# theovincent/iS-DQN

Hardware: AMD Instinct MI355X
Metric: gradient-steps/sec (batch=256, K=9, 84x84x4) (higher is better)
Workload: dtype bf16x3 (split-bf16 MFMA operands hi+lo, fp32 accumulate)

## Files before the change

### is-dqn_amd/csrc/conv_img.h

```cpp
#pragma once
#include "net_problems.h"

namespace isdqn {

__device__ __forceinline__ int column_slot(int c16) { return c16 < 4 ? 8 + c16 : (c16 < 12 ? c16 - 4 : c16); }
struct PixelOrder {
    int strips;
    int n_full;
    int full_w;
    FastDiv d_h8, d_rem, d_w;
    PixelOrder() : strips(0), n_full(0), full_w(0) {}
    PixelOrder(int H, int W, bool use_strips) : strips(use_strips ? 1 : 0), n_full(H * 8 * (W / 8)), full_w(8 * (W / 8)) {
        d_h8 = FastDiv((uint32_t)(H * 8));
        d_rem = FastDiv((uint32_t)(W % 8 ? W % 8 : 1));
        d_w = FastDiv((uint32_t)W);
    }
    __device__ __forceinline__ void map(int n, int& y, int& x) const {
        uint32_t a, b;
        if (!strips) {
            d_w.divmod((uint32_t)n, a, b);
            y = (int)a; x = (int)b;
        } else if (n < n_full) {
            d_h8.divmod((uint32_t)n, a, b);
            y = (int)(b >> 3); x = (int)(a * 8 + (b & 7));
// ... 553 lines not shown
#undef ISDQN_STAMP
#undef ISDQN_ABLATED
}

template <int MT, int PASSES, bool U8, int KG = 1>
static int launch_conv_fwd_img(const ConvImgParams& p, hipStream_t st) {
    using T = ConvImgTraits<MT, PASSES, U8>;
    const int lds = (KG * 2 * T::A_STAGE + T::B_PLANES * p.plane_elems) * 2;
    static LdsConfigured configured;
    if (int rc = ensure_dynamic_lds(&conv_fwd_img_kernel<MT, PASSES, U8, KG>, lds, configured)) return rc;
    ISDQN_REPORT_OCCUPANCY((&conv_fwd_img_kernel<MT, PASSES, U8, KG>), GEMM_THREADS * KG, lds, p.n_img * p.tiles_per_img);
    hipLaunchKernelGGL((conv_fwd_img_kernel<MT, PASSES, U8, KG>), dim3(p.n_img * p.tiles_per_img), dim3(GEMM_THREADS * KG), lds,
                       st, p);
    ISDQN_HIP_CHECK(hipGetLastError());
    return ISDQN_OK;
}

static inline int conv_img_geometry(const ConvGeom& g, bool u8, int stack, int b_planes, int mt, int a_planes, int& R,
                                    int& Wp, int& plane_elems, int pixel_pitch = 0) {
    int rows_per_tile = g.npix <= 128 ? g.hout : ((128 + g.wout - 2) / g.wout + 1);
    if (rows_per_tile > g.hout) rows_per_tile = g.hout;
    R = g.stride * (rows_per_tile - 1) + g.ksz;
    if (u8) {
        Wp = ((g.wout - 1) * g.stride + g.ksz + 7) / 8 * 8;
        plane_elems = stack * R * Wp;
    } else {
        Wp = (g.wout - 1) * g.stride + g.ksz;
        plane_elems = R * Wp * (pixel_pitch ? pixel_pitch : g.cin_p);
    }
    const int a_stage = a_planes * (mt * 16) * 48;
    return (2 * a_stage + b_planes * plane_elems) * 2;
}


struct ConvWgradImgParams {
    ConvGeom g;
    const float* dz;
    const float* in;
    FrameSrc fs;
    float* slabs;
    float scale;
    int n_img, G;
    int n_col_groups, NC;
    int R, Wp;
    int PPin;
    int in_plane;
    int PA, npix_pad;
    int dz_plane;
    FastDiv d_ncg;
    FastDiv d_chunk, d_Wp, d_R, d_dzchunk, d_npixpad;
    int prefetch;
    long long* stamps;
};
template <int WV> struct WgradPrefetch { static constexpr int DZ = 1024 / (64 * WV), IN = WV == 4 ? 6 : 5, DZ_U8 = 1792 / (64 * WV); };

template <bool U8, int PASSES, int NTHR = GEMM_THREADS>
__device__ __forceinline__ void fill_input_image(__bf16* img, int plane_elems, const ConvGeom& g, const FrameSrc& fs,
                                                 const float* in, int j, int row_base, int R, int Wp, int PP, int tid,
                                                 const FastDiv& d_chunk, const FastDiv& d_Wp, const FastDiv& d_R) {
    constexpr int FILL_BATCH = 8;
    if constexpr (U8) {
        fill_frames_u8<NTHR>(img, fs, j, row_base, -g.pad, R, Wp, tid, d_chunk);
    } else {
        fill_image_s8<NTHR, (PASSES >= 3 ? 2 : 1), FILL_BATCH>(img, plane_elems, in + (int64_t)j * g.hin * g.win * g.cin_p, g.hin, g.win, g.cin_p,
                                                               row_base, -g.pad, R, Wp, PP, tid, d_chunk, d_Wp);
    }
}

__device__ __forceinline__ bf16x8 tr_frag(const __bf16* a0, const __bf16* a1) {
    s16x4 lo = __builtin_amdgcn_ds_read_tr16_b64_v4i16((LDS_AS s16x4*)a0);
    s16x4 hi = __builtin_amdgcn_ds_read_tr16_b64_v4i16((LDS_AS s16x4*)a1);
    s16x8 r = __builtin_shufflevector(lo, hi, 0, 1, 2, 3, 4, 5, 6, 7);
    return __builtin_bit_cast(bf16x8, r);
}

template <int MT, int NTW, int PASSES, bool U8, int WV = 4>
__global__ __launch_bounds__(64 * WV) void conv_wgrad_img_kernel(const ConvWgradImgParams p) {
    ISDQN_EMPTY_KERNEL_RETURN
    constexpr int NTHR = 64 * WV;
    constexpr int A_PLANES = PASSES >= 2 ? 2 : 1;
    constexpr int B_PLANES = (PASSES >= 3) ? 2 : 1;
    extern __shared__ __attribute__((aligned(16))) char smem_raw[];
    __bf16* dzi = reinterpret_cast<__bf16*>(smem_raw);
    __bf16* img = dzi + A_PLANES * p.dz_plane;
    const ConvGeom& g = p.g;
    const int tid = threadIdx.x, lane = tid & 63, wave = tid >> 6;
#if defined(ISDQN_DEV)
#define WG_STAMP(i)                                                                                   \
    if (p.stamps != nullptr && threadIdx.x == 0) {                                                   \
        p.stamps[(int64_t)blockIdx.x * 8 + (i)] = (long long)__builtin_amdgcn_s_memtime();            \
        if ((i) == 0) p.stamps[(int64_t)blockIdx.x * 8 + 7] = (long long)__builtin_amdgcn_s_memrealtime(); \
    }
#else
#define WG_STAMP(i)
#endif
    WG_STAMP(0);
    uint32_t ig_u, cg_u;
    p.d_ncg.divmod(blockIdx.x, ig_u, cg_u);
    const int cg = (int)cg_u, ig = (int)ig_u;
    const int j0 = ig * p.G, j1 = min(p.n_img, j0 + p.G);
    const int grp = lane >> 4, li = lane & 15, q = li >> 2, pq = li & 3;

    int col_off[NTW];
#pragma unroll
    for (int t = 0; t < NTW; ++t) {
        const int c0 = cg * p.NC + (wave + WV * t) * 16;
        if constexpr (U8) {
            const int c = c0 >> 6, ky0 = (c0 >> 3) & 7;
            col_off[t] = (c * p.R + ky0 + (pq >> 1)) * p.Wp + 4 * (pq & 1);
        } else {
            uint32_t tap, ci, ky, kx;
            g.d_cinp.divmod((uint32_t)(c0 < g.K ? c0 : 0), tap, ci);
            g.d_ksz.divmod(tap, ky, kx);
            col_off[t] = ((int)ky * p.Wp + (int)kx) * p.PPin + (int)ci + 4 * pq;
        }
    }

    f32x4 acc[MT][NTW];
#pragma unroll
    for (int mt = 0; mt < MT; ++mt)
#pragma unroll
        for (int t = 0; t < NTW; ++t) mfma_init(acc[mt][t]);

    const int nsteps = p.npix_pad / GEMM_BK;
    auto k_steps = [&]() {
        for (int ks = 0; ks < nsteps; ++ks) {
            int pixoff[2], arow[2];
#pragma unroll
            for (int h = 0; h < 2; ++h) {
                int kp = ks * GEMM_BK + tr_row(8 * grp + 4 * h + q);
                arow[h] = kp * p.PA + 4 * pq;
                kp = kp < g.npix ? kp : g.npix - 1;
                uint32_t oy, ox;
                g.d_wout.divmod((uint32_t)kp, oy, ox);
                pixoff[h] = U8 ? ((int)oy * g.stride * p.Wp + (int)ox * g.stride)
                               : ((int)oy * g.stride * p.Wp + (int)ox * g.stride) * p.PPin;
            }
            bf16x8 fa_hi[MT], fa_lo[MT];
#pragma unroll
            for (int mt = 0; mt < MT; ++mt) {
                fa_hi[mt] = tr_frag(dzi + arow[0] + mt * 16, dzi + arow[1] + mt * 16);
                if constexpr (PASSES >= 2)
                    fa_lo[mt] = tr_frag(dzi + p.dz_plane + arow[0] + mt * 16, dzi + p.dz_plane + arow[1] + mt * 16);
            }
#pragma unroll
            for (int t = 0; t < NTW; ++t) {
                const __bf16* b0 = img + pixoff[0] + col_off[t];
                const __bf16* b1 = img + pixoff[1] + col_off[t];
                bf16x8 fb_hi = tr_frag(b0, b1), fb_lo;
                if constexpr (PASSES >= 3) fb_lo = tr_frag(b0 + p.in_plane, b1 + p.in_plane);
#pragma unroll
// ... 31 lines not shown
                if (j == j0) { WG_STAMP(2); } else if (j == j0 + 1) { WG_STAMP(4); }
            }
        }
    }
    if (!staged)
    for (int j = j0; j < j1; ++j) {
        __syncthreads();
        bool dz_done = false;
        if constexpr (U8) {
            if (p.prefetch) {
                ImagePrefetch<WgradPrefetch<WV>::DZ_U8> ra;
                request_image_s8<NTHR>(ra, p.dz + (int64_t)j * g.npix * g.cout_p, 1, g.npix, g.cout_p, 0, 0, 1, p.npix_pad, p.PA, tid,
                                       p.d_dzchunk, p.d_npixpad);
                fill_input_image<U8, PASSES, NTHR>(img, p.in_plane, g, p.fs, p.in, j, -g.pad, p.R, p.Wp, p.PPin, tid, p.d_chunk, p.d_Wp, p.d_R);
                commit_image_s8<A_PLANES>(dzi, p.dz_plane, ra);
                dz_done = true;
            }
        }
        if (!dz_done) {
            fill_image_s8<NTHR, A_PLANES, 8>(dzi, p.dz_plane, p.dz + (int64_t)j * g.npix * g.cout_p, 1, g.npix, g.cout_p, 0, 0, 1, p.npix_pad,
                                             p.PA, tid, p.d_dzchunk, p.d_npixpad);
            fill_input_image<U8, PASSES, NTHR>(img, p.in_plane, g, p.fs, p.in, j, -g.pad, p.R, p.Wp, p.PPin, tid, p.d_chunk, p.d_Wp, p.d_R);
        }
        __syncthreads();
        if (j == j0) { WG_STAMP(1); } else if (j == j0 + 1) { WG_STAMP(3); }
        k_steps();
        if (j == j0) { WG_STAMP(2); } else if (j == j0 + 1) { WG_STAMP(4); }
    }

    float* slab = p.slabs + (int64_t)ig * g.cout_p * g.K;
#pragma unroll
    for (int mt = 0; mt < MT; ++mt)
#pragma unroll
        for (int t = 0; t < NTW; ++t) {
            const int col = cg * p.NC + (wave + WV * t) * 16 + li;
#pragma unroll
            for (int r = 0; r < 4; ++r) {
                const int row = mt * 16 + grp * 4 + r;
#if !defined(ISDQN_NO_STREAMING)
                if (row < g.cout_p && col < g.K) __builtin_nontemporal_store(acc[mt][t][r] * p.scale, (ISDQN_GLOBAL float*)(slab + (int64_t)row * g.K + col));
#else
                if (row < g.cout_p && col < g.K) slab[(int64_t)row * g.K + col] = acc[mt][t][r] * p.scale;
#endif
            }
        }
#if defined(ISDQN_DEV)
    if (p.stamps != nullptr) {
        __builtin_amdgcn_s_waitcnt(0);
        WG_STAMP(5);
    }
#endif
#undef WG_STAMP
}

template <int MT, int NTW, int PASSES, bool U8, int WV = 4>
static int launch_conv_wgrad_img(const ConvWgradImgParams& p, int n_img_groups, hipStream_t st) {
    constexpr int A_PLANES = PASSES >= 2 ? 2 : 1;
    constexpr int B_PLANES = (PASSES >= 3) ? 2 : 1;
    const int lds = (A_PLANES * p.dz_plane + B_PLANES * p.in_plane) * 2;
    static LdsConfigured configured;
    if (int rc = ensure_dynamic_lds(&conv_wgrad_img_kernel<MT, NTW, PASSES, U8, WV>, lds, configured)) return rc;
    ISDQN_REPORT_OCCUPANCY((&conv_wgrad_img_kernel<MT, NTW, PASSES, U8, WV>), 64 * WV, lds, n_img_groups * p.n_col_groups);
    ConvWgradImgParams q = p;
    q.prefetch = 0;
#if !defined(ISDQN_WGRAD_NO_PREFETCH)
    if (!U8 && p.G >= 2 && p.npix_pad * (p.g.cout_p / 8) <= WgradPrefetch<WV>::DZ * 64 * WV &&
        p.R * p.Wp * (p.g.cin_p / 8) <= WgradPrefetch<WV>::IN * 64 * WV)
        q.prefetch = 1;
#if !defined(ISDQN_WGRAD_NO_U8_DZ)
    if (U8 && p.npix_pad * (p.g.cout_p / 8) <= WgradPrefetch<WV>::DZ_U8 * 64 * WV) q.prefetch = 1;
#endif
#endif
    hipLaunchKernelGGL((conv_wgrad_img_kernel<MT, NTW, PASSES, U8, WV>), dim3(n_img_groups * p.n_col_groups),
                       dim3(64 * WV), lds, st, q);
    ISDQN_HIP_CHECK(hipGetLastError());
    return ISDQN_OK;
}


struct ConvDgradImgParams {
    ConvGeom g;
    const float* W;
    const float* dz;
    const float* z_in;
    const float *gamma, *beta;
    int c_in;
    float* dz_in;
    float* part;
    int n_img, T, Kc;
    int Hd, Wd, PPd, bt;
    FastDiv d_chunk, d_Wd, d_T;
    long long* stamps;
    int dz_plane;
    int tiles_per_img;
    int cls_tile_start[5];
    PixelOrder cls_order[4];
    int n_classes;
};

template <int MT, int PASSES, int NT = 2>
__global__ __launch_bounds__(GEMM_THREADS, 2) void conv_dgrad_img_kernel(const ConvDgradImgParams p) {
    ISDQN_EMPTY_KERNEL_RETURN
    constexpr int BM = MT * 16;
    constexpr int A_PLANES = PASSES >= 2 ? 2 : 1;
    constexpr int B_PLANES = PASSES >= 3 ? 2 : 1;
    using GA = TileGeom<BM, true>;
    constexpr int A_STAGE = A_PLANES * GA::ELEMS;
    extern __shared__ __attribute__((aligned(16))) char smem_raw[];
    __bf16* a_stage = reinterpret_cast<__bf16*>(smem_raw);
    __bf16* img = a_stage + 2 * A_STAGE;
    __shared__ float s_part[4][3][64];
    const ConvGeom& g = p.g;
    const int tid = threadIdx.x, lane = tid & 63, wave = tid >> 6, grp = lane >> 4;
#if defined(ISDQN_DEV)
#define ISDQN_STAMP(i)                                                                               \
    if (p.stamps != nullptr && threadIdx.x == 0) {                                                  \
        p.stamps[(int64_t)blockIdx.x * 8 + (i)] = (long long)__builtin_amdgcn_s_memtime();           \
        if ((i) == 0) p.stamps[(int64_t)blockIdx.x * 8 + 7] = (long long)__builtin_amdgcn_s_memrealtime(); \
    }
#define ISDQN_ABLATED(bit) ((p.ablate & (bit)) != 0)
#else
#define ISDQN_STAMP(i)
#define ISDQN_ABLATED(bit) (false)
#endif
    ISDQN_STAMP(0);

    int j, tl;
// ... 298 lines not shown
                    out[mt][r] = ok ? rstd * (gg[mt][r] - m1 - xh[mt][r] * m2) : 0.f;
                    dbias[mt][r] += out[mt][r];
                }
        } else {
#pragma unroll
            for (int mt = 0; mt < MT; ++mt)
#pragma unroll
                for (int r = 0; r < 4; ++r) {
                    const bool ok = pix_ok[nt] && (mt * 16 + grp * 4 + r) < p.c_in;
                    out[mt][r] = (ok && zv[mt][r] > 0.f) ? acc[mt][nt][r] : 0.f;
                    dbias[mt][r] += out[mt][r];
                }
        }
        if (pix_ok[nt]) {
#pragma unroll
            for (int mt = 0; mt < MT; ++mt) {
                const int ch0 = mt * 16 + grp * 4;
                if (ch0 < g.cin_p)
                    s8_store_quad_paired(p.dz_in + pixel * g.cin_p, ch0, out[mt][0], out[mt][1], out[mt][2], out[mt][3]);
            }
        }
    }
#pragma unroll
    for (int mt = 0; mt < MT; ++mt)
#pragma unroll
        for (int r = 0; r < 4; ++r) {
            dg[mt][r] = row16_sum(dg[mt][r]);
            db[mt][r] = row16_sum(db[mt][r]);
            dbias[mt][r] = row16_sum(dbias[mt][r]);
            if ((lane & 15) == 0) {
                const int ch = mt * 16 + grp * 4 + r;
                s_part[wave][0][ch] = dg[mt][r];
                s_part[wave][1][ch] = db[mt][r];
                s_part[wave][2][ch] = dbias[mt][r];
            }
        }
    __syncthreads();
    for (int i = tid; i < 3 * g.cin_p; i += GEMM_THREADS) {
        const int which = (i >= g.cin_p) + (i >= 2 * g.cin_p), c = i - which * g.cin_p;
        p.part[((int64_t)blockIdx.x * 3 + which) * g.cin_p + c] =
            s_part[0][which][c] + s_part[1][which][c] + s_part[2][which][c] + s_part[3][which][c];
    }
    ISDQN_STAMP(4);
#if defined(ISDQN_DEV)
    if (p.stamps != nullptr) {
        __builtin_amdgcn_s_waitcnt(0);
        ISDQN_STAMP(5);
    }
#endif
#undef ISDQN_STAMP
#undef ISDQN_ABLATED
}

constexpr int REDUCE_MAX_JOBS = 4;
struct ReduceJobs {
    const float* part[REDUCE_MAX_JOBS];
    float* out[REDUCE_MAX_JOBS];
    int n_rows[REDUCE_MAX_JOBS], width[REDUCE_MAX_JOBS];
    int block_start[REDUCE_MAX_JOBS + 1];
    int n;
};
__global__ __launch_bounds__(256) void reduce_rows_kernel(const ReduceJobs jobs) {
    ISDQN_EMPTY_KERNEL_RETURN
    __shared__ float s_red[32][8];
    int job = 0;
#pragma unroll
    for (int i = 1; i < REDUCE_MAX_JOBS; ++i)
        if (i < jobs.n && (int)blockIdx.x >= jobs.block_start[i]) job = i;
    const float* __restrict__ part = jobs.part[job];
    float* __restrict__ out = jobs.out[job];
    const int n_rows = jobs.n_rows[job], width = jobs.width[job];
    const int col = ((int)blockIdx.x - jobs.block_start[job]) * 8 + (threadIdx.x & 7), rl = threadIdx.x >> 3;
    float s = 0.f;
    if (col < width) {
        int r = rl;
        for (; r + 7 * 32 < n_rows; r += 8 * 32) {
            float v[8];
#pragma unroll
            for (int u = 0; u < 8; ++u) v[u] = part[(int64_t)(r + u * 32) * width + col];
#pragma unroll
            for (int u = 0; u < 8; ++u) s += v[u];
        }
        for (; r < n_rows; r += 32) s += part[(int64_t)r * width + col];
    }
    s_red[rl][threadIdx.x & 7] = s;
    __syncthreads();
    if (rl == 0 && col < width) {
        float t = 0.f;
#pragma unroll
        for (int k = 0; k < 32; ++k) t += s_red[k][threadIdx.x & 7];
        out[col] = t;
    }
}

template <int MT, int PASSES, int NT = 2>
static int launch_conv_dgrad_img(const ConvDgradImgParams& p, hipStream_t st) {
    constexpr int A_PLANES = PASSES >= 2 ? 2 : 1;
    constexpr int B_PLANES = PASSES >= 3 ? 2 : 1;
    using GA = TileGeom<MT * 16, true>;
    const int lds = (2 * A_PLANES * GA::ELEMS + B_PLANES * p.dz_plane) * 2;
    static LdsConfigured configured;
    if (int rc = ensure_dynamic_lds(&conv_dgrad_img_kernel<MT, PASSES, NT>, lds, configured)) return rc;
    ISDQN_REPORT_OCCUPANCY((&conv_dgrad_img_kernel<MT, PASSES, NT>), GEMM_THREADS, lds, p.n_img * p.tiles_per_img);
    hipLaunchKernelGGL((conv_dgrad_img_kernel<MT, PASSES, NT>), dim3(p.n_img * p.tiles_per_img), dim3(GEMM_THREADS), lds, st, p);
    ISDQN_HIP_CHECK(hipGetLastError());
    return ISDQN_OK;
}

}
```

### is-dqn_amd/csrc/net_kernels.hip

```cpp
#include <stdarg.h>
#include <stdlib.h>

#include <algorithm>
#include <type_traits>
#include <vector>
#include <atomic>

#include "conv_img.h"
#include "conv_u8_pair.h"
#include "conv_s8_pair.h"
#include "munchausen.h"
#include "hl_gauss.h"
#include "quantile.h"
#include "net_plan.h"
#include "net_problems.h"

namespace isdqn {

__device__ inline double pow_int(double b, int t) {
    double r = 1.0, x = b;
    for (unsigned u = (unsigned)t; u != 0; u >>= 1) {
        if (u & 1u) r *= x;
        x *= x;
    }
// ... 1344 lines not shown
    else if (Cp <= 128) LAUNCH_SMALL(32);
    else if (Cp <= 256) LAUNCH_SMALL(64);
    else {
        ISDQN_REQUIRE(Cp <= 256 * LN_WIDE_MAX_COLS, ISDQN_ERR_UNSUPPORTED, "hidden dense width above 4096");
        nb = rows < LN_MAX_BLOCKS ? rows : LN_MAX_BLOCKS;
        hipLaunchKernelGGL(ln_bwd_wide_kernel, dim3(nb), dim3(256), 0, st, da, z, gamma, beta, rows, C, Cp, dz, part);
    }
#undef LAUNCH_SMALL
    ISDQN_HIP_CHECK(hipGetLastError());
    *n_blocks_out = nb;
    return ISDQN_OK;
}

template <int BM, int PASSES>
static int launch_conv_dgrad(const Layer& l, const float* wmir, const float* dz, float* da, int n_img,
                             hipStream_t st) {
    ConvDgrad<BM, PASSES> p;
    p.g = conv_geom(l);
    p.W = wmir + l.w_off;
    p.dz = dz; p.da = da; p.n_img = n_img;
    p.T = l.ksz / l.stride;
    p.Kc = p.T * p.T * l.cout_p;
    p.n_classes = l.stride * l.stride;
    int acc = 0;
    for (int c = 0; c < p.n_classes; ++c) {
        int cy = c / l.stride, cx = c % l.stride;
        int Ha = (l.hin - cy + l.stride - 1) / l.stride, Wb = (l.win - cx + l.stride - 1) / l.stride;
        p.tile_start[c] = acc;
        p.cls_d_hw[c] = FastDiv((uint32_t)(Ha * Wb));
        p.cls_d_w[c] = FastDiv((uint32_t)Wb);
        acc += ceil_div(n_img * Ha * Wb, 128);
    }
    p.tile_start[p.n_classes] = acc;
    return launch_gemm(p, acc, st);
}

template <int PASSES, bool U8>
static int launch_conv_wgrad(const Layer& l, const NetInput& in, const float* act_in, const float* dz, float* slabs,
                             int n_img, hipStream_t st) {
    ConvWgrad<PASSES, U8> p;
    p.g = conv_geom(l);
    p.n_pix = n_img * l.npix;
    p.DZ = MatSrc{dz, l.cout_p, p.n_pix, l.cout_p, 1};
    p.in = act_in;
    p.fs = FrameSrc{in.frames, in.frame_stride, in.frame_ids, l.cin, in.paired_B, l.hin, l.win, in.id_pitch, in.id_off};
    p.slabs = slabs;
    p.scale = U8 ? (1.0f / 255.0f) : 1.0f;
    p.tiles_n = ceil_div(l.K, 64);
    int ksteps = ceil_div(p.n_pix, GEMM_BK);
    p.steps_per_split = ceil_div(ksteps, l.gw_slabs);
    p.splits = ceil_div(ksteps, p.steps_per_split);
    return launch_gemm(p, p.tiles_n * p.splits, st);
}
static int conv_wgrad_img(const Layer& l, bool x3, const NetInput& in, const float* act_in, const float* dz, float* slabs,
                          int n_img, hipStream_t st, int* slabs_out) {
    *slabs_out = 0;
    if (!l.wgi_ntw || n_img != 0 && ceil_div(n_img, l.wgi_G) > l.gw_slabs) return ISDQN_OK;
    ConvWgradImgParams wp;
    wp.g = conv_geom(l);
    const int passes = x3 ? (l.is_u8 ? 2 : 3) : 1;
    const int mt = l.cout_p <= 32 ? 2 : 4;
    int lds_unused_R, Wp, plane;
    conv_img_geometry(wp.g, l.is_u8, l.cin, 1, mt, 1, lds_unused_R, Wp, plane);
    wp.R = l.stride * (l.hout - 1) + l.ksz;
    wp.Wp = Wp;
    wp.PPin = l.cin_p;
    for (int pad = 0; pad <= 24; pad += 8)
        if ((l.stride * (l.cin_p + pad)) % 32 == 16) { wp.PPin = l.cin_p + pad; break; }
    wp.in_plane = l.is_u8 ? l.cin * wp.R * Wp : wp.R * Wp * wp.PPin;
    wp.PA = l.cout_p + (l.cout_p % 32 == 0 ? 16 : 8);
    wp.npix_pad = round_up(l.npix, 32);
    wp.dz_plane = wp.npix_pad * wp.PA;
    const int lds = ((passes >= 2 ? 2 : 1) * wp.dz_plane + (passes >= 3 ? 2 : 1) * wp.in_plane) * 2;
    if (lds > 150 * 1024 || (l.is_u8 && (l.win < 8 || l.cin > 4))) return ISDQN_OK;
    wp.d_chunk = FastDiv((uint32_t)(l.is_u8 ? Wp / 8 : l.cin_p / 8));
    wp.d_Wp = FastDiv((uint32_t)Wp);
    wp.d_R = FastDiv((uint32_t)wp.R);
    wp.d_dzchunk = FastDiv((uint32_t)(l.cout_p / 8));
    wp.d_npixpad = FastDiv((uint32_t)wp.npix_pad);
    wp.dz = dz; wp.in = act_in;
    wp.fs = FrameSrc{in.frames, in.frame_stride, in.frame_ids, l.cin, in.paired_B, l.hin, l.win, in.id_pitch, in.id_off};
    wp.slabs = slabs;
    wp.scale = l.is_u8 ? (1.0f / 255.0f) : 1.0f;
    wp.n_img = n_img; wp.G = l.wgi_G;
    wp.NC = 64 * l.wgi_ntw;
    wp.n_col_groups = l.K / wp.NC;
    wp.d_ncg = FastDiv((uint32_t)wp.n_col_groups);
    {
        char tag[32];
        snprintf(tag, sizeof(tag), "wgrad:%s", l.name);
        wp.stamps = stamps_for(tag);
    }
    const int groups = ceil_div(n_img, l.wgi_G);
    *slabs_out = groups;
#define WGI(MT_, NTW_, P_, U_) return launch_conv_wgrad_img<MT_, NTW_, P_, U_>(wp, groups, st)
#define WGI8(MT_, NTW_, P_, U_) return launch_conv_wgrad_img<MT_, NTW_, P_, U_, 8>(wp, groups, st)
    if (l.is_u8) {
        if (mt == 2) { if (l.wgi_ntw == 4) { if (passes == 2) WGI(2, 4, 2, true); else WGI(2, 4, 1, true); }
                       if (l.wgi_ntw == 2) { if (passes == 2) WGI(2, 2, 2, true); else WGI(2, 2, 1, true); } }
        else         { if (l.wgi_ntw == 4) { if (passes == 2) WGI(4, 4, 2, true); else WGI(4, 4, 1, true); }
                       if (l.wgi_ntw == 2) { if (passes == 2) WGI(4, 2, 2, true); else WGI(4, 2, 1, true); } }
    } else {
        if (mt == 2) { if (l.wgi_ntw == 4) { if (passes == 3) WGI(2, 4, 3, false); else WGI(2, 4, 1, false); }
                       if (l.wgi_ntw == 3) { if (passes == 3) WGI(2, 3, 3, false); else WGI(2, 3, 1, false); }
                       if (l.wgi_ntw == 2) { if (passes == 3) WGI(2, 2, 3, false); else WGI(2, 2, 1, false); } }
        else         {
                       static const bool w4 = ISDQN_DEV_ENV("ISDQN_WGRAD_4WAVES");
                       if (l.wgi_ntw == 8 && !w4) { if (passes == 3) WGI8(4, 4, 3, false); else WGI8(4, 4, 1, false); }
                       if (l.wgi_ntw == 9) { if (passes == 3) WGI(4, 9, 3, false); else WGI(4, 9, 1, false); }
                       if (l.wgi_ntw == 8) { if (passes == 3) WGI(4, 8, 3, false); else WGI(4, 8, 1, false); }
                       if (l.wgi_ntw == 4) { if (passes == 3) WGI(4, 4, 3, false); else WGI(4, 4, 1, false); }
                       if (l.wgi_ntw == 3) { if (passes == 3) WGI(4, 3, 3, false); else WGI(4, 3, 1, false); }
                       if (l.wgi_ntw == 2) { if (passes == 3) WGI(4, 2, 3, false); else WGI(4, 2, 1, false); } }
    }
#undef WGI
#undef WGI8
    *slabs_out = 0;
    return ISDQN_OK;
}

static void add_reduce_job(ReduceJobs& jobs, const float* part, int n_rows, int width, float* out) {
    const int i = jobs.n++;
    jobs.part[i] = part; jobs.out[i] = out; jobs.n_rows[i] = n_rows; jobs.width[i] = width;
    jobs.block_start[i + 1] = jobs.block_start[i] + ceil_div(width, 8);
}

static int conv_dgrad_img(const Layer& l, const Layer& below, bool x3, const float* params, const float* wmir, const float* dz, float* ws,
                          int n_img, hipStream_t st, bool* done, ReduceJobs* jobs) {
    *done = false;
    if (!l.dgi_tiles || below.part_rows < n_img * l.dgi_tiles) return ISDQN_OK;
    ConvDgradImgParams dp;
    dp.g = conv_geom(l);
    dp.W = wmir + l.w_off;
    dp.dz = dz;
    dp.z_in = ws + below.z_off;
    dp.gamma = below.has_ln ? params + below.g_off : nullptr;
    dp.beta = below.has_ln ? params + below.be_off : nullptr;
    dp.c_in = below.out_f;
    dp.dz_in = ws + below.dz_off;
    dp.part = ws + below.part_off;
    dp.n_img = n_img;
    dp.T = l.ksz / l.stride;
    dp.Kc = dp.T * dp.T * l.cout_p;
#if defined(ISDQN_DGRAD_WIDE_BORDER)
    dp.bt = dp.T - 1;
#else
    dp.bt = dp.T - 1 - l.pad / l.stride > 0 ? dp.T - 1 - l.pad / l.stride : 0;
#endif
    const int need_h = (l.hin - 1 + l.pad) / l.stride + 1, need_w = (l.win - 1 + l.pad) / l.stride + 1;
    dp.Hd = dp.bt + (l.hout > need_h ? l.hout : need_h);
    dp.Wd = dp.bt + (l.wout > need_w ? l.wout : need_w);
    dp.PPd = l.cout_p + ((16 - l.cout_p % 32) + 32) % 32;
    dp.dz_plane = dp.Hd * dp.Wd * dp.PPd;
    dp.d_chunk = FastDiv((uint32_t)(l.cout_p / 8));
    dp.d_Wd = FastDiv((uint32_t)dp.Wd);
    dp.d_T = FastDiv((uint32_t)dp.T);
    {
        char tag[32];
        snprintf(tag, sizeof(tag), "dgrad:%s", l.name);
        dp.stamps = stamps_for(tag);
    }
    dp.n_classes = l.stride * l.stride;
    int acc = 0;
    for (int c = 0; c < dp.n_classes; ++c) {
        int cy = c / l.stride, cx = c % l.stride;
        int Ha = (l.hin - cy + l.stride - 1) / l.stride, Wb = (l.win - cx + l.stride - 1) / l.stride;
        dp.cls_tile_start[c] = acc;
        dp.cls_order[c] = PixelOrder(Ha, Wb, Ha * Wb <= 128);
        acc += ceil_div(Ha * Wb, l.dgi_tile_pix);
    }
    dp.cls_tile_start[dp.n_classes] = acc;
// ... 527 lines not shown

struct WgradJob {
    int layer = -1;
    hipStream_t stream = nullptr;
    hipEvent_t wait = nullptr;
    const float* dz = nullptr;
    int dz_ld = 0;
};

static int dense_wgrad_fused_adam(const LearnCtx& c, const Layer& l, const float* act_in, const WgradJob& j) {
    const MatSrc A{j.dz, j.dz_ld, c.B, l.out_p, 1};
    const MatSrc Bm{act_in, l.in_p, c.B, l.in_p, 1};
    AdamFuse af{c.params + l.w_off, c.adam_m + l.w_off, c.adam_v + l.w_off, c.ws + c.P.adam_tab_off,
                c.cfg->learning_rate, c.cfg->adam_b1, c.cfg->adam_b2, c.cfg->adam_eps,
                c.grad_out ? c.grad_out + l.w_off : nullptr, c.ws + c.P.wsplit_off + l.w_off, c.update ? 1 : 0};
    if (l.is_head)
        return c.x3 ? launch_plain<64, 64, 2, 2, true, true, 3, true, false, true, 2>(A, nullptr, 0, Bm, nullptr, l.in_p, l.out_p, l.in_p, c.B, 1, 0,
                                                                                      j.stream, &af)
                    : launch_plain<64, 64, 2, 2, true, true, 1, true, false, true, 2>(A, nullptr, 0, Bm, nullptr, l.in_p, l.out_p, l.in_p, c.B, 1, 0,
                                                                                      j.stream, &af);
    return c.x3 ? launch_plain<64, 64, 2, 2, true, true, 3, true, false, true, DZ_S8 | 2>(A, nullptr, 0, Bm, nullptr, l.in_p, l.out_p, l.in_p, c.B, 1,
                                                                                          0, j.stream, &af)
                : launch_plain<64, 64, 2, 2, true, true, 1, true, false, true, DZ_S8 | 2>(A, nullptr, 0, Bm, nullptr, l.in_p, l.out_p, l.in_p, c.B, 1,
                                                                                          0, j.stream, &af);
}

static int weight_gradient(const LearnCtx& c, const WgradJob& j, AdamList* adam) {
    const Layer& l = c.P.L[j.layer];
    float* ws = c.ws;
    const float* act_in = j.layer > 0 ? ws + c.P.L[j.layer - 1].act_off : nullptr;
    int w_slabs, rc;
    if (l.is_head && c.hc_S && c.ss) {
        w_slabs = effective_splits(c.B, l.gw_slabs);
    } else if (l.kind == 0) {
        rc = conv_wgrad(l, c.x3, c.in, act_in, j.dz, ws + l.gw_off, c.B, j.stream, &w_slabs);
        if (rc) return rc;
    } else {
        w_slabs = effective_splits(c.B, l.gw_slabs);
        if (w_slabs == 1 && !l.in_unpadded_ld) return dense_wgrad_fused_adam(c, l, act_in, j);
        rc = dense_wgrad(l, c.x3, c.in, act_in, j.dz, j.dz_ld, ws + l.gw_off, c.B, j.stream);
        if (rc) return rc;
    }
    adam[c.ss && j.stream == c.wst ? 1 : 0].add(l.w_off, l.w_size, ws + l.gw_off, w_slabs, l.w_size);
    return ISDQN_OK;
}

#if !defined(ISDQN_FORK_LATE_MAX_B)
#define ISDQN_FORK_LATE_MAX_B 768
#endif
struct BackwardSchedule {
    const LearnCtx& c;
    AdamList* const adam;
    const bool tail_swap, fork_late;
    bool prio_pending, head_pending;
    hipEvent_t head_event = nullptr;
    bool forked = false, layer0_chained = false;
    WgradJob deferred;

    BackwardSchedule(const LearnCtx& ctx, AdamList* lists)
        : c(ctx), adam(lists), tail_swap(ctx.ss && ctx.P.n_layers >= 3 && !ctx.P.L[1].is_head),
          fork_late(ctx.ss != nullptr && ctx.P.L[0].kind != 2 && ctx.B <= ISDQN_FORK_LATE_MAX_B),
          prio_pending(ctx.batch->priorities_ready != nullptr), head_pending(ctx.hc_S && ctx.ss) {}

    bool wgrad_on_side(int i) const { return c.ss && !c.P.L[i].is_head && (tail_swap ? i != 1 : i > 0); }
    hipStream_t wgrad_stream(int i) const { return wgrad_on_side(i) || (c.P.L[i].is_head && c.hc_S) ? c.wst : c.st; }
    bool forks_after_dgrad(int i) const { return wgrad_on_side(i) && c.P.L[i].kind == 1 && i > 0; }
    bool forks_before_dgrad(int i) const { return wgrad_on_side(i) && !forks_after_dgrad(i) && !(i == 0 && layer0_chained); }
    bool adam_on_side() const { return c.ss && forked && tail_swap; }

    int signal_priorities() {
        if (prio_pending) {
            prio_pending = false;
            ISDQN_HIP_CHECK(hipEventRecord((hipEvent_t)c.batch->priorities_ready, c.st));
        }
        return ISDQN_OK;
    }
    int run_head_tail(hipStream_t s) {
        if (!head_pending) return ISDQN_OK;
        head_pending = false;
        return head_chain_tail(c, s);
    }
    int begin() {
        if (!c.ss)
            if (int rc = signal_priorities()) return rc;
        if (fork_late && head_pending) {
            head_event = next_event(c.ss);
            ISDQN_HIP_CHECK(hipEventRecord(head_event, c.st));
        }
        return ISDQN_OK;
    }
    int fork(hipStream_t side) {
        if (int rc = chain(c.ss, c.st, side)) return rc;
        if (int rc = signal_priorities()) return rc;
        forked = true;
        return deferred.layer < 0 ? run_head_tail(side) : ISDQN_OK;
    }
    int fork_after_dgrad(WgradJob& job, bool* defer) {
        if (!fork_late) {
            if (int rc = chain(c.ss, c.st, job.stream)) return rc;
            if (int rc = signal_priorities()) return rc;
            forked = true;
            return run_head_tail(job.stream);
        }
        if (head_event != nullptr && head_pending) {
            ISDQN_HIP_CHECK(hipStreamWaitEvent(job.stream, head_event, 0));
            if (int rc = run_head_tail(job.stream)) return rc;
        }
        job.wait = next_event(c.ss);
        ISDQN_HIP_CHECK(hipEventRecord(job.wait, c.st));
        *defer = true;
        forked = true;
        return signal_priorities();
    }
    int chain_layer0() {
        if (int rc = chain(c.ss, c.st, c.wst)) return rc;
        forked = layer0_chained = true;
        return run_head_tail(c.wst);
    }
    int flush() {
        if (deferred.layer < 0) return ISDQN_OK;
        const WgradJob j = deferred;
        deferred.layer = -1;
        ISDQN_HIP_CHECK(hipStreamWaitEvent(j.stream, j.wait, 0));
        if (int rc = run_head_tail(j.stream)) return rc;
        return weight_gradient(c, j, adam);
    }
    int finish() {
        if (int rc = flush()) return rc;
        if (int rc = run_head_tail(c.st)) return rc;
        return signal_priorities();
    }
};

static bool dense_dgrad_ln_applies(const Layer& l, const Layer& below, int B) {
    return l.kind == 1 && below.kind != 1 && below.cout_p == 64 && !l.in_unpadded_ld && below.part_rows >= ceil_div(B, 128) * below.npix;
}
static int dense_dgrad_ln(const LearnCtx& c, const Layer& l, const Layer& below, const float* dz, int dz_ld, ReduceJobs* red) {
    float* ws = c.ws;
    const int B = c.B;
    auto launch = [&](auto prob) {
        prob.A = MatSrc{dz, dz_ld, B, l.out_p, 1};
        prob.B = MatSrc{c.wmir() + l.w_off, l.in_p, l.out_f, l.in_p, 1};
        prob.z = ws + below.z_off;
        prob.gamma = below.has_ln ? c.params + below.g_off : nullptr;
        prob.beta = below.has_ln ? c.params + below.be_off : nullptr;
        prob.dz_out = ws + below.dz_off;
        prob.part = ws + below.part_off;
        prob.ldc = l.in_p; prob.M = B; prob.N = l.in_p; prob.K = l.out_p; prob.c_in = below.out_f;
        prob.tiles_m = ceil_div(B, decltype(prob)::BM); prob.tiles_n = l.in_p / 64;
        return launch_gemm(prob, prob.tiles_m * prob.tiles_n, c.st);
    };
    static const bool no_kg = ISDQN_DEV_ENV("ISDQN_NO_KGROUPS");
    const bool kg2 = !no_kg && ceil_div(B, 128) * (l.in_p / 64) <= 256 && l.out_p % 64 == 0;
    int rc;
#if defined(ISDQN_DGRAD64)
    (void)kg2;
    rc = c.x3 ? launch(DenseDgradLN<3, 64>{}) : launch(DenseDgradLN<1, 64>{});
    constexpr int DG_BM = 64;
#else
    if (kg2) rc = c.x3 ? launch(DenseDgradLN<3, 128, 2>{}) : launch(DenseDgradLN<1, 128, 2>{});
    else rc = c.x3 ? launch(DenseDgradLN<3, 128>{}) : launch(DenseDgradLN<1, 128>{});
    constexpr int DG_BM = 128;
#endif
    if (rc) return rc;
    add_reduce_job(*red, ws + below.part_off, ceil_div(B, DG_BM) * (l.in_p / 64), 3 * below.out_p, ws + below.red_off);
// ... 18 lines not shown
    return dense_dgrad(l, c.x3, c.wmir(), dz, dz_ld, da, c.B, narrow, c.st);
}

static int learn_backward(const LearnCtx& c, BackwardSchedule& sched, AdamList* adam, ReduceJobs* red) {
    const Plan& P = c.P;
    float* ws = c.ws;
    const int B = c.B;
    int rc;
    const float* dz_cur = ws + P.dout_off;
    int dz_ld = P.nlog_p;
    bool dz_fused = false;
    for (int i = P.n_layers - 1; i >= 0; --i) {
        const Layer& l = P.L[i];
        if (l.is_head) {
            adam[c.hc_S && c.ss ? 1 : 0].add(l.b_off, l.out_p, ws + P.dbh_off, 1, 0);
        } else {
            dz_cur = ws + l.dz_off;
            dz_ld = l.out_p;
            if (c.hc_S && i == P.n_layers - 2) {
                add_ln_bias_entries(adam[0], l, ws + l.part_off, c.hc_wg, 3 * (int64_t)l.out_p);
            } else if (dz_fused) {
                add_ln_bias_entries(adam[0], l, ws + l.red_off, 1, 0);
            } else {
                int nb = 0;
                rc = ln_bwd(l, c.params, ws + P.da_off, ws + l.z_off, l.kind != 1 ? B * l.npix : B, ws + l.dz_off, ws + l.part_off, &nb, c.st);
                if (rc) return rc;
                add_ln_bias_entries(adam[0], l, ws + l.part_off, nb, 3 * (int64_t)l.out_p);
            }
        }
        if (l.kind == 2) {
            rc = impala_backward(P, c.cfg, c.x3, c.params, c.adam_m, c.adam_v, c.wmir(), ws, B, c.grad_out, c.update, c.st);
            if (rc) return rc;
            continue;
        }
        WgradJob job;
        job.layer = i; job.stream = sched.wgrad_stream(i); job.dz = dz_cur; job.dz_ld = dz_ld;
        if (sched.forks_before_dgrad(i)) {
            rc = sched.fork(job.stream);
            if (rc) return rc;
        }
        dz_fused = false;
        if (i > 0) {
            rc = data_gradient(c, i, dz_cur, dz_ld, &dz_fused, red);
            if (rc) return rc;
        }
        rc = sched.flush();
        if (rc) return rc;
        bool defer = false;
        if (sched.forks_after_dgrad(i)) {
            rc = sched.fork_after_dgrad(job, &defer);
            if (rc) return rc;
        }
        if (sched.tail_swap && i == 1 && dz_fused) {
            rc = sched.chain_layer0();
            if (rc) return rc;
        }
        if (defer) {
            sched.deferred = job;
        } else {
            rc = weight_gradient(c, job, adam);
            if (rc) return rc;
        }
    }
    return sched.finish();
}

static int learn_optimizer(const LearnCtx& c, const BackwardSchedule& sched, const AdamList* adam, const ReduceJobs& red) {
    auto run_adam = [&](const AdamList& list, hipStream_t s) {
        return list.launch(s, c.P, c.cfg, c.params, c.adam_m, c.adam_v, c.ws, c.grad_out, c.update);
    };
    int rc;
    if (sched.adam_on_side()) {
        rc = run_adam(adam[1], c.wst);
        if (rc) return rc;
    } else if (c.ss) {
        rc = chain(c.ss, c.wst, c.st);
        if (rc) return rc;
    }
    if (red.n > 0) {
        hipLaunchKernelGGL(reduce_rows_kernel, dim3(red.block_start[red.n]), dim3(256), 0, c.st, red);
        ISDQN_HIP_CHECK(hipGetLastError());
    }
    rc = run_adam(adam[0], c.st);
    if (rc) return rc;
    return sched.adam_on_side() ? chain(c.ss, c.wst, c.st) : run_adam(adam[1], c.st);
}

static int learn_or_loss(const isdqn_net_config* cfg, float* params, float* adam_m, float* adam_v, int32_t* adam_count,
                         const isdqn_batch* batch, float* losses, float* loss_accum, float* q_values, float* targets,
                         double* priorities, void* workspace, void* stream, bool learn, float* grad_out,
                         const float* target_params = nullptr, const HeadSel* sel = nullptr, bool update = true) {
    int rc;
    const Plan* Pp = cached_plan(cfg, &rc);
    if (!Pp) return rc;
    const Plan& P = *Pp;
    ISDQN_REQUIRE(params && batch && losses && workspace, ISDQN_ERR_ARG, "null pointer");
    ISDQN_REQUIRE(batch->B == P.B, ISDQN_ERR_SHAPE, "batch->B != cfg->batch_size");
    ISDQN_REQUIRE(batch->action && batch->reward && batch->terminal, ISDQN_ERR_ARG, "null batch field");
    rc = check_input(cfg, batch->frames, batch->frame_stride, batch->frame_ids, batch->state);
    if (rc) return rc;
    if (cfg->arch == ISDQN_ARCH_FC) ISDQN_REQUIRE(batch->next_state != nullptr, ISDQN_ERR_ARG, "fc needs next_state");
    if (learn && update) ISDQN_REQUIRE(adam_m && adam_v && adam_count, ISDQN_ERR_ARG, "null optimizer state");
    if (learn && !update) {
        ISDQN_REQUIRE(grad_out != nullptr, ISDQN_ERR_ARG, "a gradient-only pass needs grad_out");
        adam_m = params;
        adam_v = params;
    }
    if (P.bn) {
        ISDQN_REQUIRE(target_params == nullptr || (learn && !update), ISDQN_ERR_UNSUPPORTED,
                      "BatchNorm networks: separate target parameters only in gradient-only passes (the reference's DQN cannot run with "
                      "batch_norm, dqn.py:86)");
        ISDQN_REQUIRE(target_params == nullptr || cfg->double_q == 0, ISDQN_ERR_UNSUPPORTED,
                      "BatchNorm networks: double_q with separate target parameters is not defined (no statistics for an online forward "
                      "of the next states)");
        ISDQN_REQUIRE(target_params == nullptr || !P.munchausen, ISDQN_ERR_UNSUPPORTED,
                      "BatchNorm networks: Munchausen targets with separate target parameters are not defined (no statistics for a target "
                      "forward of the states)");
        return bn_learn_or_loss(cfg, P, params, adam_m, adam_v, adam_count, batch, losses, loss_accum, q_values, targets, priorities,
                                (float*)workspace, (hipStream_t)stream, learn, grad_out, update, target_params, sel);
    }
    const int B = P.B, K = sel ? sel->K : P.K;
    const int on0 = sel ? sel->on0 : P.oh, tg0 = sel ? sel->tg0 : 0;
    if (sel) ISDQN_REQUIRE(sel->K >= 1 && on0 >= 0 && tg0 >= 0 && on0 + K <= P.n_heads && tg0 + K <= P.n_heads && K <= P.K, ISDQN_ERR_ARG,
                           "head selection outside the network's heads");
// ... 254 lines not shown
```

Before: 4264.

## Fuse layer-1 and layer-0 wgrad with row reduction into one paired kernel

Turns the image-wgrad kernel into a device body and adds a paired kernel with 512-thread blocks. Block ranges in one launch run layer 1's wgrad, layer 0's u8 wgrad, and optionally the reduce_rows jobs. The backward schedule now launches this pair on the main stream at the tail and drops the separate layer-0 wgrad, reduce launch and cross-stream chaining. This cuts launch count and stream sync at the end of the backward pass, at the cost of 8-wave blocks sized to the larger LDS footprint of the two layers and a reworked Adam ordering.

Result: no change. 4301, median of 6 (+0.9%).

```diff
diff --git a/is-dqn_amd/csrc/conv_img.h b/is-dqn_amd/csrc/conv_img.h
--- a/is-dqn_amd/csrc/conv_img.h
+++ b/is-dqn_amd/csrc/conv_img.h
@@ -629,7 +629,7 @@
     int prefetch;
     long long* stamps;
 };
-template <int WV> struct WgradPrefetch { static constexpr int DZ = 1024 / (64 * WV), IN = WV == 4 ? 6 : 5, DZ_U8 = 1792 / (64 * WV); };
+template <int WV> struct WgradPrefetch { static constexpr int DZ = 1024 / (64 * WV), IN = WV == 4 ? 6 : 5, DZ_U8 = (1792 + 64 * WV - 1) / (64 * WV); };
 
 template <bool U8, int PASSES, int NTHR = GEMM_THREADS>
 __device__ __forceinline__ void fill_input_image(__bf16* img, int plane_elems, const ConvGeom& g, const FrameSrc& fs,
@@ -651,9 +651,8 @@
     return __builtin_bit_cast(bf16x8, r);
 }
 
-template <int MT, int NTW, int PASSES, bool U8, int WV = 4>
-__global__ __launch_bounds__(64 * WV) void conv_wgrad_img_kernel(const ConvWgradImgParams p) {
-    ISDQN_EMPTY_KERNEL_RETURN
+template <int MT, int NTW, int PASSES, bool U8, int WV>
+__device__ __forceinline__ void conv_wgrad_img_body(const ConvWgradImgParams& p, const int bid) {
     constexpr int NTHR = 64 * WV;
     constexpr int A_PLANES = PASSES >= 2 ? 2 : 1;
     constexpr int B_PLANES = (PASSES >= 3) ? 2 : 1;
@@ -665,15 +664,15 @@
 #if defined(ISDQN_DEV)
 #define WG_STAMP(i)                                                                                   \
     if (p.stamps != nullptr && threadIdx.x == 0) {                                                   \
-        p.stamps[(int64_t)blockIdx.x * 8 + (i)] = (long long)__builtin_amdgcn_s_memtime();            \
-        if ((i) == 0) p.stamps[(int64_t)blockIdx.x * 8 + 7] = (long long)__builtin_amdgcn_s_memrealtime(); \
+        p.stamps[(int64_t)bid * 8 + (i)] = (long long)__builtin_amdgcn_s_memtime();            \
+        if ((i) == 0) p.stamps[(int64_t)bid * 8 + 7] = (long long)__builtin_amdgcn_s_memrealtime(); \
     }
 #else
 #define WG_STAMP(i)
 #endif
     WG_STAMP(0);
     uint32_t ig_u, cg_u;
-    p.d_ncg.divmod(blockIdx.x, ig_u, cg_u);
+    p.d_ncg.divmod((uint32_t)bid, ig_u, cg_u);
     const int cg = (int)cg_u, ig = (int)ig_u;
     const int j0 = ig * p.G, j1 = min(p.n_img, j0 + p.G);
     const int grp = lane >> 4, li = lane & 15, q = li >> 2, pq = li & 3;
@@ -811,27 +810,116 @@
 #endif
 #undef WG_STAMP
 }
+template <int MT, int NTW, int PASSES, bool U8, int WV = 4>
+__global__ __launch_bounds__(64 * WV) void conv_wgrad_img_kernel(const ConvWgradImgParams p) {
+    ISDQN_EMPTY_KERNEL_RETURN
+    conv_wgrad_img_body<MT, NTW, PASSES, U8, WV>(p, (int)blockIdx.x);
+}
+constexpr int REDUCE_MAX_JOBS = 4;
+struct ReduceJobs {
+    const float* part[REDUCE_MAX_JOBS];
+    float* out[REDUCE_MAX_JOBS];
+    int n_rows[REDUCE_MAX_JOBS], width[REDUCE_MAX_JOBS];
+    int block_start[REDUCE_MAX_JOBS + 1];
+    int n;
+};
+template <int NTHR>
+__device__ __forceinline__ void reduce_rows_body(const ReduceJobs& jobs, const int bid) {
+    __shared__ float s_red[32][8];
+    const bool active = NTHR == 256 || threadIdx.x < 256;
+    int job = 0;
+#pragma unroll
+    for (int i = 1; i < REDUCE_MAX_JOBS; ++i)
+        if (i < jobs.n && bid >= jobs.block_start[i]) job = i;
+    const float* __restrict__ part = jobs.part[job];
+    float* __restrict__ out = jobs.out[job];
+    const int n_rows = jobs.n_rows[job], width = jobs.width[job];
+    const int col = (bid - jobs.block_start[job]) * 8 + (threadIdx.x & 7), rl = threadIdx.x >> 3;
+    float s = 0.f;
+    if (active && col < width) {
+        int r = rl;
+        for (; r + 7 * 32 < n_rows; r += 8 * 32) {
+            float v[8];
+#pragma unroll
+            for (int u = 0; u < 8; ++u) v[u] = part[(int64_t)(r + u * 32) * width + col];
+#pragma unroll
+            for (int u = 0; u < 8; ++u) s += v[u];
+        }
+        for (; r < n_rows; r += 32) s += part[(int64_t)r * width + col];
+    }
+    if (active) s_red[rl][threadIdx.x & 7] = s;
+    __syncthreads();
+    if (rl == 0 && col < width) {
+        float t = 0.f;
+#pragma unroll
+        for (int k = 0; k < 32; ++k) t += s_red[k][threadIdx.x & 7];
+        out[col] = t;
+    }
+}
+__global__ __launch_bounds__(256) void reduce_rows_kernel(const ReduceJobs jobs) {
+    ISDQN_EMPTY_KERNEL_RETURN
+    reduce_rows_body<256>(jobs, (int)blockIdx.x);
+}
+
+template <int MT_A, int NTW_A, int PASSES_A, bool U8_A, int MT_B, int NTW_B, int PASSES_B, bool U8_B>
+__global__ __launch_bounds__(512) void conv_wgrad_img_pair_kernel(const ConvWgradImgParams pa, const int n_a, const ConvWgradImgParams pb,
+                                                                  const int n_b, const ReduceJobs red) {
+    ISDQN_EMPTY_KERNEL_RETURN
+    const int bid = (int)blockIdx.x;
+    if (bid < n_a) conv_wgrad_img_body<MT_A, NTW_A, PASSES_A, U8_A, 8>(pa, bid);
+    else if (bid < n_a + n_b) conv_wgrad_img_body<MT_B, NTW_B, PASSES_B, U8_B, 8>(pb, bid - n_a);
+    else reduce_rows_body<512>(red, bid - n_a - n_b);
+}
+
+template <int PASSES>
+static inline int conv_wgrad_img_lds(const ConvWgradImgParams& p) {
+    constexpr int A_PLANES = PASSES >= 2 ? 2 : 1;
+    constexpr int B_PLANES = (PASSES >= 3) ? 2 : 1;
+    return (A_PLANES * p.dz_plane + B_PLANES * p.in_plane) * 2;
+}
+template <bool U8, int WV>
+static inline int conv_wgrad_img_prefetch(const ConvWgradImgParams& p) {
+#if !defined(ISDQN_WGRAD_NO_PREFETCH)
+    if (!U8 && p.G >= 2 && p.npix_pad * (p.g.cout_p / 8) <= WgradPrefetch<WV>::DZ * 64 * WV &&
+        p.R * p.Wp * (p.g.cin_p / 8) <= WgradPrefetch<WV>::IN * 64 * WV)
+        return 1;
+#if !defined(ISDQN_WGRAD_NO_U8_DZ)
+    if (U8 && p.npix_pad * (p.g.cout_p / 8) <= WgradPrefetch<WV>::DZ_U8 * 64 * WV) return 1;
+#endif
+#endif
+    return 0;
+}
 
 template <int MT, int NTW, int PASSES, bool U8, int WV = 4>
 static int launch_conv_wgrad_img(const ConvWgradImgParams& p, int n_img_groups, hipStream_t st) {
-    constexpr int A_PLANES = PASSES >= 2 ? 2 : 1;
-    constexpr int B_PLANES = (PASSES >= 3) ? 2 : 1;
-    const int lds = (A_PLANES * p.dz_plane + B_PLANES * p.in_plane) * 2;
+    const int lds = conv_wgrad_img_lds<PASSES>(p);
     static LdsConfigured configured;
     if (int rc = ensure_dynamic_lds(&conv_wgrad_img_kernel<MT, NTW, PASSES, U8, WV>, lds, configured)) return rc;
     ISDQN_REPORT_OCCUPANCY((&conv_wgrad_img_kernel<MT, NTW, PASSES, U8, WV>), 64 * WV, lds, n_img_groups * p.n_col_groups);
     ConvWgradImgParams q = p;
-    q.prefetch = 0;
-#if !defined(ISDQN_WGRAD_NO_PREFETCH)
-    if (!U8 && p.G >= 2 && p.npix_pad * (p.g.cout_p / 8) <= WgradPrefetch<WV>::DZ * 64 * WV &&
-        p.R * p.Wp * (p.g.cin_p / 8) <= WgradPrefetch<WV>::IN * 64 * WV)
-        q.prefetch = 1;
-#if !defined(ISDQN_WGRAD_NO_U8_DZ)
-    if (U8 && p.npix_pad * (p.g.cout_p / 8) <= WgradPrefetch<WV>::DZ_U8 * 64 * WV) q.prefetch = 1;
-#endif
-#endif
+    q.prefetch = conv_wgrad_img_prefetch<U8, WV>(p);
     hipLaunchKernelGGL((conv_wgrad_img_kernel<MT, NTW, PASSES, U8, WV>), dim3(n_img_groups * p.n_col_groups),
                        dim3(64 * WV), lds, st, q);
+    ISDQN_HIP_CHECK(hipGetLastError());
+    return ISDQN_OK;
+}
+template <int MT_A, int NTW_A, int PASSES_A, bool U8_A, int MT_B, int NTW_B, int PASSES_B, bool U8_B>
+static int launch_conv_wgrad_img_pair(const ConvWgradImgParams& a, int groups_a, const ConvWgradImgParams& b, int groups_b, const ReduceJobs* red,
+                                      hipStream_t st) {
+    auto kern = &conv_wgrad_img_pair_kernel<MT_A, NTW_A, PASSES_A, U8_A, MT_B, NTW_B, PASSES_B, U8_B>;
+    const int lds_a = conv_wgrad_img_lds<PASSES_A>(a), lds_b = conv_wgrad_img_lds<PASSES_B>(b);
+    const int lds = lds_a > lds_b ? lds_a : lds_b;
+    const int n_a = groups_a * a.n_col_groups, n_b = groups_b * b.n_col_groups;
+    static LdsConfigured configured;
+    if (int rc = ensure_dynamic_lds(kern, lds, configured)) return rc;
+    ReduceJobs rj = {};
+    if (red != nullptr) rj = *red;
+    const int n_r = rj.block_start[rj.n];
+    ISDQN_REPORT_OCCUPANCY(kern, 512, lds, n_a + n_b + n_r);
+    ConvWgradImgParams qa = a, qb = b;
+    qa.prefetch = conv_wgrad_img_prefetch<U8_A, 8>(a);
+    qb.prefetch = conv_wgrad_img_prefetch<U8_B, 8>(b);
+    hipLaunchKernelGGL(kern, dim3(n_a + n_b + n_r), dim3(512), lds, st, qa, n_a, qb, n_b, rj);
     ISDQN_HIP_CHECK(hipGetLastError());
     return ISDQN_OK;
 }
@@ -1236,47 +1324,6 @@
 #undef ISDQN_ABLATED
 }
 
-constexpr int REDUCE_MAX_JOBS = 4;
-struct ReduceJobs {
-    const float* part[REDUCE_MAX_JOBS];
-    float* out[REDUCE_MAX_JOBS];
-    int n_rows[REDUCE_MAX_JOBS], width[REDUCE_MAX_JOBS];
-    int block_start[REDUCE_MAX_JOBS + 1];
-    int n;
-};
-__global__ __launch_bounds__(256) void reduce_rows_kernel(const ReduceJobs jobs) {
-    ISDQN_EMPTY_KERNEL_RETURN
-    __shared__ float s_red[32][8];
-    int job = 0;
-#pragma unroll
-    for (int i = 1; i < REDUCE_MAX_JOBS; ++i)
-        if (i < jobs.n && (int)blockIdx.x >= jobs.block_start[i]) job = i;
-    const float* __restrict__ part = jobs.part[job];
-    float* __restrict__ out = jobs.out[job];
-    const int n_rows = jobs.n_rows[job], width = jobs.width[job];
-    const int col = ((int)blockIdx.x - jobs.block_start[job]) * 8 + (threadIdx.x & 7), rl = threadIdx.x >> 3;
-    float s = 0.f;
-    if (col < width) {
-        int r = rl;
-        for (; r + 7 * 32 < n_rows; r += 8 * 32) {
-            float v[8];
-#pragma unroll
-            for (int u = 0; u < 8; ++u) v[u] = part[(int64_t)(r + u * 32) * width + col];
-#pragma unroll
-            for (int u = 0; u < 8; ++u) s += v[u];
-        }
-        for (; r < n_rows; r += 32) s += part[(int64_t)r * width + col];
-    }
-    s_red[rl][threadIdx.x & 7] = s;
-    __syncthreads();
-    if (rl == 0 && col < width) {
-        float t = 0.f;
-#pragma unroll
-        for (int k = 0; k < 32; ++k) t += s_red[k][threadIdx.x & 7];
-        out[col] = t;
-    }
-}
-
 template <int MT, int PASSES, int NT = 2>
 static int launch_conv_dgrad_img(const ConvDgradImgParams& p, hipStream_t st) {
     constexpr int A_PLANES = PASSES >= 2 ? 2 : 1;
diff --git a/is-dqn_amd/csrc/net_kernels.hip b/is-dqn_amd/csrc/net_kernels.hip
--- a/is-dqn_amd/csrc/net_kernels.hip
+++ b/is-dqn_amd/csrc/net_kernels.hip
@@ -1420,11 +1420,9 @@
     p.splits = ceil_div(ksteps, p.steps_per_split);
     return launch_gemm(p, p.tiles_n * p.splits, st);
 }
-static int conv_wgrad_img(const Layer& l, bool x3, const NetInput& in, const float* act_in, const float* dz, float* slabs,
-                          int n_img, hipStream_t st, int* slabs_out) {
-    *slabs_out = 0;
-    if (!l.wgi_ntw || n_img != 0 && ceil_div(n_img, l.wgi_G) > l.gw_slabs) return ISDQN_OK;
-    ConvWgradImgParams wp;
+static bool conv_wgrad_img_params(const Layer& l, bool x3, const NetInput& in, const float* act_in, const float* dz, float* slabs, int n_img,
+                                  ConvWgradImgParams& wp) {
+    if (!l.wgi_ntw || n_img != 0 && ceil_div(n_img, l.wgi_G) > l.gw_slabs) return false;
     wp.g = conv_geom(l);
     const int passes = x3 ? (l.is_u8 ? 2 : 3) : 1;
     const int mt = l.cout_p <= 32 ? 2 : 4;
@@ -1440,7 +1438,7 @@
     wp.npix_pad = round_up(l.npix, 32);
     wp.dz_plane = wp.npix_pad * wp.PA;
     const int lds = ((passes >= 2 ? 2 : 1) * wp.dz_plane + (passes >= 3 ? 2 : 1) * wp.in_plane) * 2;
-    if (lds > 150 * 1024 || (l.is_u8 && (l.win < 8 || l.cin > 4))) return ISDQN_OK;
+    if (lds > 150 * 1024 || (l.is_u8 && (l.win < 8 || l.cin > 4))) return false;
     wp.d_chunk = FastDiv((uint32_t)(l.is_u8 ? Wp / 8 : l.cin_p / 8));
     wp.d_Wp = FastDiv((uint32_t)Wp);
     wp.d_R = FastDiv((uint32_t)wp.R);
@@ -1459,6 +1457,15 @@
         snprintf(tag, sizeof(tag), "wgrad:%s", l.name);
         wp.stamps = stamps_for(tag);
     }
+    return true;
+}
+static int conv_wgrad_img(const Layer& l, bool x3, const NetInput& in, const float* act_in, const float* dz, float* slabs,
+                          int n_img, hipStream_t st, int* slabs_out) {
+    *slabs_out = 0;
+    ConvWgradImgParams wp;
+    if (!conv_wgrad_img_params(l, x3, in, act_in, dz, slabs, n_img, wp)) return ISDQN_OK;
+    const int passes = x3 ? (l.is_u8 ? 2 : 3) : 1;
+    const int mt = l.cout_p <= 32 ? 2 : 4;
     const int groups = ceil_div(n_img, l.wgi_G);
     *slabs_out = groups;
 #define WGI(MT_, NTW_, P_, U_) return launch_conv_wgrad_img<MT_, NTW_, P_, U_>(wp, groups, st)
@@ -1485,6 +1492,24 @@
 #undef WGI8
     *slabs_out = 0;
     return ISDQN_OK;
+}
+static bool conv_wgrad_img_pair_forms(const Layer& l1, const Layer& l0) {
+    static const bool w4 = ISDQN_DEV_ENV("ISDQN_WGRAD_4WAVES");
+    return !w4 && l1.kind == 0 && l0.kind == 0 && !l1.is_u8 && l0.is_u8 && l1.cout_p > 32 && l0.cout_p <= 32 && l1.wgi_ntw == 8 && l0.wgi_ntw == 4;
+}
+static int conv_wgrad_img_pair(const Layer& l1, const Layer& l0, bool x3, const NetInput& in, const float* act0, const float* dz1, const float* dz0,
+                               float* ws, int n_img, const ReduceJobs* red, hipStream_t st, int* slabs1, int* slabs0, bool* fused) {
+    *fused = false;
+    if (!conv_wgrad_img_pair_forms(l1, l0)) return ISDQN_OK;
+    ConvWgradImgParams p1, p0;
+    if (!conv_wgrad_img_params(l1, x3, in, act0, dz1, ws + l1.gw_off, n_img, p1) ||
+        !conv_wgrad_img_params(l0, x3, in, nullptr, dz0, ws + l0.gw_off, n_img, p0))
+        return ISDQN_OK;
+    *fused = true;
+    *slabs1 = ceil_div(n_img, l1.wgi_G);
+    *slabs0 = ceil_div(n_img, l0.wgi_G);
+    return x3 ? launch_conv_wgrad_img_pair<4, 4, 3, false, 2, 2, 2, true>(p1, *slabs1, p0, *slabs0, red, st)
+              : launch_conv_wgrad_img_pair<4, 4, 1, false, 2, 2, 1, true>(p1, *slabs1, p0, *slabs0, red, st);
 }
 
 static void add_reduce_job(ReduceJobs& jobs, const float* part, int n_rows, int width, float* out) {
@@ -2118,21 +2143,30 @@
     const LearnCtx& c;
     AdamList* const adam;
     const bool tail_swap, fork_late;
+    const bool expect_pair;
     bool prio_pending, head_pending;
     hipEvent_t head_event = nullptr;
     bool forked = false, layer0_chained = false;
+    bool tail_paired = false;
+    bool sums_ride = false;
     WgradJob deferred;
 
     BackwardSchedule(const LearnCtx& ctx, AdamList* lists)
         : c(ctx), adam(lists), tail_swap(ctx.ss && ctx.P.n_layers >= 3 && !ctx.P.L[1].is_head),
           fork_late(ctx.ss != nullptr && ctx.P.L[0].kind != 2 && ctx.B <= ISDQN_FORK_LATE_MAX_B),
+          expect_pair(may_pair_tail() && conv_wgrad_img_pair_forms(ctx.P.L[1], ctx.P.L[0]) && ctx.P.L[1].dgi_tiles != 0),
           prio_pending(ctx.batch->priorities_ready != nullptr), head_pending(ctx.hc_S && ctx.ss) {}
 
-    bool wgrad_on_side(int i) const { return c.ss && !c.P.L[i].is_head && (tail_swap ? i != 1 : i > 0); }
+    bool wgrad_on_side(int i) const { return c.ss && !c.P.L[i].is_head && (tail_swap ? i != 1 : i > 0) && !(tail_paired && i == 0); }
     hipStream_t wgrad_stream(int i) const { return wgrad_on_side(i) || (c.P.L[i].is_head && c.hc_S) ? c.wst : c.st; }
-    bool forks_after_dgrad(int i) const { return wgrad_on_side(i) && c.P.L[i].kind == 1 && i > 0; }
+    bool forks_after_dgrad(int i) const { return wgrad_on_side(i) && (c.P.L[i].kind == 1 || expect_pair) && i > 0; }
     bool forks_before_dgrad(int i) const { return wgrad_on_side(i) && !forks_after_dgrad(i) && !(i == 0 && layer0_chained); }
     bool adam_on_side() const { return c.ss && forked && tail_swap; }
+    bool may_pair_tail() const {
+        static const bool off = ISDQN_DEV_ENV("ISDQN_NO_WGRAD_PAIR");
+        constexpr int PAIR_TAIL_MAX_B = 256;
+        return tail_swap && fork_late && c.B <= PAIR_TAIL_MAX_B && !off;
+    }
 
     int signal_priorities() {
         if (prio_pending) {
@@ -2177,6 +2211,23 @@
         *defer = true;
         forked = true;
         return signal_priorities();
+    }
+    int pair_tail(const ReduceJobs* red, bool* paired) {
+        *paired = false;
+        if (!expect_pair) return ISDQN_OK;
+        static const bool own_sums = ISDQN_DEV_ENV("ISDQN_NO_SUMS_RIDER");
+        if (own_sums || red->n == 0) red = nullptr;
+        const Layer &l1 = c.P.L[1], &l0 = c.P.L[0];
+        int slabs1 = 0, slabs0 = 0;
+        if (int rc = conv_wgrad_img_pair(l1, l0, c.x3, c.in, c.ws + l0.act_off, c.ws + l1.dz_off, c.ws + l0.dz_off, c.ws, c.B, red, c.st, &slabs1, &slabs0,
+                                         paired))
+            return rc;
+        if (!*paired) return ISDQN_OK;
+        tail_paired = true;
+        sums_ride = red != nullptr;
+        adam[0].add(l1.w_off, l1.w_size, c.ws + l1.gw_off, slabs1, l1.w_size);
+        adam[0].add(l0.w_off, l0.w_size, c.ws + l0.gw_off, slabs0, l0.w_size);
+        return ISDQN_OK;
     }
     int chain_layer0() {
         if (int rc = chain(c.ss, c.st, c.wst)) return rc;
@@ -2301,9 +2352,13 @@
             if (rc) return rc;
         }
         if (sched.tail_swap && i == 1 && dz_fused) {
-            rc = sched.chain_layer0();
+            bool paired = false;
+            rc = sched.pair_tail(red, &paired);
             if (rc) return rc;
-        }
+            if (!paired) rc = sched.chain_layer0();
+            if (rc) return rc;
+        }
+        if (sched.tail_paired) continue;
         if (defer) {
             sched.deferred = job;
         } else {
@@ -2319,6 +2374,23 @@
         return list.launch(s, c.P, c.cfg, c.params, c.adam_m, c.adam_v, c.ws, c.grad_out, c.update);
     };
     int rc;
+    if (sched.tail_paired) {
+        const bool side = sched.adam_on_side();
+        if (side) {
+            rc = run_adam(adam[1], c.wst);
+            if (rc) return rc;
+        }
+        if (red.n > 0 && !sched.sums_ride) {
+            hipLaunchKernelGGL(reduce_rows_kernel, dim3(red.block_start[red.n]), dim3(256), 0, c.st, red);
+            ISDQN_HIP_CHECK(hipGetLastError());
+        }
+        rc = chain(c.ss, c.wst, c.st);
+        if (rc) return rc;
+        if (side) return run_adam(adam[0], c.st);
+        AdamList all = adam[0];
+        all.e.insert(all.e.end(), adam[1].e.begin(), adam[1].e.end());
+        return run_adam(all, c.st);
+    }
     if (sched.adam_on_side()) {
         rc = run_adam(adam[1], c.wst);
         if (rc) return rc;
```
